# lemerleau/RAFFT

Hardware: AMD Instinct MI355X
Metric: sequences/sec (whole node) on benchmark set, beam N=100; kcal/mol MAE vs CPU (higher is better)
Workload: dtype f32 FFT -> exact int counts, f64 scores, i32 dcal energies

## Files before the change

### rafft_amd/csrc/rafft_device.h

```cpp
#pragma once
#include <hip/hip_runtime.h>
#include <stdint.h>

#define RAFFT_MAX_LEN 32768

struct SmallT {
    int16_t stack[7][7];
    int16_t mmH[7][5][5], mmI[7][5][5], mm1n[7][5][5], mm23[7][5][5], mmM[7][5][5], mmE[7][5][5];
    int16_t d5[7][5], d3[7][5];
    int32_t hairpin[31], bulge[31], interior[31];
    int32_t ml_base, ml_closing, ml_intern, ninio, max_ninio, term_au;
    int32_t lsb, pad_lsb_[3];
    uint32_t sp_key[128]; int32_t sp_e[128];
    uint32_t sp_filter[32];
    int16_t stk4[256];
};
static_assert(sizeof(SmallT) % 16 == 0, "SmallT is copied to LDS in 16-byte pieces");
__host__ __device__ inline uint32_t sp_tag(int size) { return (uint32_t)(size == 3 ? 1 : size == 4 ? 2 : 3) << 28; }
__host__ __device__ inline uint32_t sp_slot(uint32_t tagged) { return (tagged * 2654435761u) >> 25; }
__host__ __device__ inline uint32_t sp_filter_index(int size, int c5, int l5, int l3, int c3)
{
    return ((sp_tag(size) >> 28) << 8) | (uint32_t)((c5 + 3) & 3) | (uint32_t)((l5 + 3) & 3) << 2 | (uint32_t)((l3 + 3) & 3) << 4 | (uint32_t)((c3 + 3) & 3) << 6;
}
struct BigT {
// ... 229 lines not shown

__device__ inline int loop_energy_br(const SmallT *T, const BigT *B, const uint8_t *S, int L, int ci, int cj, const BrList &bl, int &g)
{
    const int k = bl.count();
    if (ci < 0) {
        int e = 0;
        for (int i = 0; i < k; i++) {
            int p, q;
            bl.get(i, p, q);
            e += e_stem(T, pair_type(S[p], S[q]), p > 0 ? (int)S[p - 1] : -1, q < L - 1 ? (int)S[q + 1] : -1, true);
        }
        return e;
    }
    const int type = pair_type(S[ci], S[cj]);
    if (k == 0) return e_hairpin(T, B, cj - ci - 1, type, S, ci, cj);
    if (k == 1) {
        int p, q;
        bl.get(0, p, q);
        return e_intloop(T, B, p - ci - 1, cj - q - 1, type, rtype(pair_type(S[p], S[q])), S[ci + 1], S[cj - 1], S[p - 1], S[q + 1], g);
    }
    int e = 0, u = cj - ci - 1;
    for (int i = 0; i < k; i++) {
        int p, q;
        bl.get(i, p, q);
        e += e_stem(T, pair_type(S[p], S[q]), S[p - 1], S[q + 1], false);
        u -= q - p + 1;
    }
    e += e_stem(T, rtype(type), S[cj - 1], S[ci + 1], false);
    return e + T->ml_closing + u * T->ml_base;
}

struct BrPrefix { const int *pe_ext, *pe_ml; const uint16_t *psp; };
__device__ inline int loop_energy_pre(const SmallT *T, const BigT *B, const uint8_t *S, int L, int ci, int cj, const BrList &bl, const BrPrefix &pf, int &g)
{
    const int k = bl.count();
    if (ci < 0) {
        int e = pf.pe_ext[bl.a1] - pf.pe_ext[bl.a0] + pf.pe_ext[bl.b1] - pf.pe_ext[bl.b0];
        if (bl.has_mid)
            e += e_stem(T, pair_type(S[bl.mp], S[bl.mq]), bl.mp > 0 ? (int)S[bl.mp - 1] : -1, bl.mq < L - 1 ? (int)S[bl.mq + 1] : -1, true);
        return e;
    }
    const int type = pair_type(S[ci], S[cj]);
    if (k == 0) return e_hairpin(T, B, cj - ci - 1, type, S, ci, cj);
    if (k == 1) {
        int p, q;
        bl.get(0, p, q);
        return e_intloop(T, B, p - ci - 1, cj - q - 1, type, rtype(pair_type(S[p], S[q])), S[ci + 1], S[cj - 1], S[p - 1], S[q + 1], g);
    }
    int e = pf.pe_ml[bl.a1] - pf.pe_ml[bl.a0] + pf.pe_ml[bl.b1] - pf.pe_ml[bl.b0];
    int u = cj - ci - 1 - ((int)pf.psp[bl.a1] - (int)pf.psp[bl.a0] + (int)pf.psp[bl.b1] - (int)pf.psp[bl.b0]);
    if (bl.has_mid) {
        e += e_stem(T, pair_type(S[bl.mp], S[bl.mq]), S[bl.mp - 1], S[bl.mq + 1], false);
        u -= bl.mq - bl.mp + 1;
    }
    e += e_stem(T, rtype(type), S[cj - 1], S[ci + 1], false);
    return e + T->ml_closing + u * T->ml_base;
}

__device__ __forceinline__ int br_lower(const uint32_t *br, int nbr, int x)
{
    int lo = 0, hi = nbr;
    while (lo < hi) {
        int mid = (lo + hi) >> 1;
        if ((int)(br[mid] & 0xffffu) < x) lo = mid + 1; else hi = mid;
    }
    return lo;
}

__device__ __forceinline__ void br_lower4(const uint32_t *br, int nbr, int x0, int x1, int x2, int x3, int &r0, int &r1, int &r2, int &r3)
{
    int a = 0, b = 0, c = 0, e = 0;
    int step = nbr > 0 ? 1 << (31 - __clz(nbr)) : 0;
    for (; step > 0; step >>= 1) {
        const int ia = a + step, ib = b + step, ic = c + step, ie = e + step;
        const int va = ia <= nbr ? (int)(br[ia - 1] & 0xffffu) : 0x7fffffff, vb = ib <= nbr ? (int)(br[ib - 1] & 0xffffu) : 0x7fffffff;
        const int vc = ic <= nbr ? (int)(br[ic - 1] & 0xffffu) : 0x7fffffff, ve = ie <= nbr ? (int)(br[ie - 1] & 0xffffu) : 0x7fffffff;
        if (va < x0) a = ia;
        if (vb < x1) b = ib;
        if (vc < x2) c = ic;
        if (ve < x3) e = ie;
    }
    r0 = a; r1 = b; r2 = c; r3 = e;
}
```

### rafft_amd/csrc/rafft_expand.hip

```cpp
#pragma once


__device__ __forceinline__ unsigned long long mask_window(const unsigned long long *X, int W, int start)
{
    if (start >= 64 * W || start <= -64) return 0ULL;
    const int q = start >> 6, bsh = start & 63;
    const unsigned long long lo = (q >= 0 && q < W) ? X[q] : 0ULL;
    const unsigned long long hi = (q + 1 >= 0 && q + 1 < W) ? X[q + 1] : 0ULL;
    return bsh ? (lo >> bsh) | (hi << (64 - bsh)) : lo;
}

template <int NT, class CodeAt>
__device__ inline void build_masks(unsigned long long *F, unsigned long long *R, int W, int n, const CodeAt &code_at, const uint16_t *pos, int tid)
{
    for (int wq = tid >> 6; wq < W; wq += NT / 64) {
        const int t = wq * 64 + (tid & 63);
        const int c0 = t < n ? code_at(t) : 0;
        const unsigned long long bA = __ballot(c0 == 1), bC = __ballot(c0 == 2), bG = __ballot(c0 == 3), bU = __ballot(c0 == 4);
        const unsigned long long bg = __ballot(t >= 1 && t < n && (int)pos[t] - (int)pos[t > 0 ? t - 1 : 0] == 1);
        if ((tid & 63) == 0) { F[0 * W + wq] = bA; F[1 * W + wq] = bC; F[2 * W + wq] = bG; F[3 * W + wq] = bU; F[4 * W + wq] = bg; }
    }
    if (NT == 64) { __builtin_amdgcn_fence(__ATOMIC_ACQ_REL, "wavefront"); __builtin_amdgcn_wave_barrier(); } else __syncthreads();
    for (int idx = tid; idx < 5 * W; idx += NT) {
        const int which = idx / W, w = idx - which * W;
// ... 874 lines not shown
        if (item >= n_items) { fetch_left = 0; continue; }
        const int nid = NT == 64 ? __builtin_amdgcn_readfirstlane(d.work[cls][item]) : d.work[cls][item];
        const int L = d.nd[nid].L;
        const int n = d.nd[nid].n, ci = d.nd[nid].ci, cj = d.nd[nid].cj, nbr = d.nd[nid].nbr;
        const int par_dcal = d.nd[nid].pdcal;
        const uint16_t *posg = d.pos + d.nd[nid].pos;
        const uint32_t *brg = d.br + d.nd[nid].br;
        const uint8_t *codes = d.codes + d.nd[nid].soff;
        const int sx0 = ci < 0 ? 0 : ci, sx1 = ci < 0 ? L : cj + 1;
        const int spad = LONGSEQ ? 0 : (int)((uintptr_t)(codes + sx0) & 3u);
        const uint8_t *Sl = LONGSEQ ? codes : (const uint8_t *)Sl_lds + spad - sx0;
        const int m = 2 * n - 1;
        const int P = next_pow2_ge(m);
        const int logP = 31 - __clz(P);
        const int Pk = LONGSEQ == 2 ? 0 : P;
        const int Kp = d.K < m ? (d.K > 0 ? d.K : 0) : m;
        ExpandRegion<CODE_LDS> g{tm};
        g.nid = nid; g.n = n; g.m = m; g.P = P; g.logP = logP; g.Kp = Kp; g.nbr = nbr; g.ci = ci; g.cj = cj; g.L = L; g.par_dcal = par_dcal;
        g.codes = codes; g.Sl = Sl;

        load_region<NT, LONGSEQ>(d, g, posg, brg, Sl_lds, sx0, sx1, spad);

        const bool direct = (NT == 64) && n <= 64 && !force_fft;
        const bool mw = !direct && LONGSEQ != 2 && (nofft || (n <= d.direct_n && P >= 128 && dbg.lag == nullptr && !force_fft &&
                        d.gc >= 0.0 && d.au >= 0.0 && d.gu >= 0.0));
        const bool ranked = m > Kp;
        const bool selected = ranked && P >= 128;
        const bool inplace = (ranked && !selected) || (dbg.lag != nullptr && !selected);
        const RegionA<LONGSEQ> A(lds, lay, P, Pk, n, nmax, selected, inplace, nofft, d, gteam);
        LagTally tally;
        if (LONGSEQ == 2 || mw) lag_values_masks<NT, PROD>(d, g, A, tally);
        else if (direct) lag_values_wave<NT, PROD>(d, g, A, tally);
        else {
            fft_correlate<NT>(g, A, tw, twN);
            lag_values_fft<NT, PROD>(d, g, A, tally);
        }

        if (selected) {
            select_lags<NT, PROD>(g, A, tally);
            report_ranking<NT>(g, A);
        } else sort_lags_inplace<NT>(g, A);

        const int C = (NT >= 256 && selected) ? max(1, min(8, NT / max(Kp, 1))) : 1;
        const bool ws_masks = PROD || (d.gc >= 0.0 && d.au >= 0.0 && d.gu >= 0.0 && !force_fft);
        if (ws_masks) {
            const int W = A.W();
            unsigned long long *F = A.slide_masks(), *R = F + MASK_F_WORDS * W;
            WsPart *parts = A.slide_parts();
            if (LONGSEQ != 2 && (!mw || A.inplace)) {
                build_masks<NT>(F, R, W, n, [&](int t) -> int { return g.code_at(t); }, pos, tid);
                ESYNC();
            }
            const uint32_t *F32 = (const uint32_t *)F, *R32 = (const uint32_t *)R;
            const int W2 = 2 * W;
            double wgc = d.gc, wau = d.au, wgu = d.gu;
            asm volatile("" : "+v"(wgc), "+v"(wau), "+v"(wgu));
            auto win = [](const uint32_t *X, int start) -> uint32_t { const int q_ = start >> 5; return __builtin_amdgcn_alignbit(X[q_ + 1], X[q_], (uint32_t)(start & 31)); };
            for (int q = tid; q < Kp * C; q += NT) {
                const int r = q / C, c = q - r * C;
                const int lagp = rk[r];
                const Diag dg = diag_of(lagp, n);
                const int ip0 = dg.ip0;
                const int lim = eligible_prefix(pos, dg.len, dg.len2, ip0, dg.jp0, d.min_hp);
                const int ca = (int)((long long)lim * c / C), ce = (int)((long long)lim * (c + 1) / C);
                const int rs0 = n - 1 - lagp + ip0;
                auto cells = [&](int k, uint32_t &pGC, uint32_t &pAU, uint32_t &pGU, uint32_t &cm) {
                    const int cs = ip0 + 32 * k, rs = rs0 + 32 * k;
                    const uint32_t fA = win(F32 + 0 * W2, cs), fC = win(F32 + 1 * W2, cs), fG = win(F32 + 2 * W2, cs), fU = win(F32 + 3 * W2, cs);
                    const uint32_t xA = win(R32 + 0 * W2, rs), xC = win(R32 + 1 * W2, rs), xG = win(R32 + 2 * W2, rs), xU = win(R32 + 3 * W2, rs);
                    pGC = d.gc != 0.0 ? ((fG & xC) | (fC & xG)) : 0u;
                    pAU = d.au != 0.0 ? ((fA & xU) | (fU & xA)) : 0u;
                    pGU = d.gu != 0.0 ? ((fG & xU) | (fU & xG)) : 0u;
                    cm = win(F32 + 4 * W2, cs) & win(R32 + 4 * W2, rs);
                    if (k == 0) cm &= ~1u;
                };
                auto span = [](int lo_, int hi_, int cb) -> uint32_t {
                    uint32_t m_ = ~0u;
                    if (lo_ > cb) m_ &= ~0u << (lo_ - cb);
                    if (hi_ < cb + 32) m_ &= (1u << (hi_ - cb)) - 1u;
                    return m_;
                };
                double mx_s = 0.0, prev = 0.0;
                int mx_nb = 0, mx_c = 0, last_c = -2, runlen = 0, mx_i = 0, mx_j = 0;
                if (ce > ca) {
                    int z = ca;
                    if (ca > 0) {
                        for (int kz = (ca - 1) >> 5;; kz--) {
                            const int cb = kz << 5;
                            uint32_t pGC, pAU, pGU, cm;
                            cells(kz, pGC, pAU, pGU, cm);
                            const uint32_t zeros = ~(pGC | pAU | pGU) & span(0, ca, cb);
                            if (zeros) { z = cb + 32 - __clz((int)zeros); break; }
                            if (cb == 0) { z = 0; break; }
                        }
                    }
                    for (int k = z >> 5; k <= (ce - 1) >> 5; k++) {
                        const int cb = k << 5;
                        uint32_t pGC, pAU, pGU, cm;
                        cells(k, pGC, pAU, pGU, cm);
                        uint32_t any = (pGC | pAU | pGU) & span(z, ce, cb);
                        while (any) {
                            const int bi = __ffs((int)any) - 1;
                            any &= any - 1u;
                            const int cc = cb + bi;
                            const double w8 = ((pGC >> bi) & 1u) ? wgc : ((pAU >> bi) & 1u) ? wau : wgu;
                            if (cc != last_c + 1) { prev = 0.0; runlen = 0; }
                            double t = w8;
                            if ((cm >> bi) & 1u) t = (prev + w8) * w8;
                            runlen++;
                            if ((C == 1 || cc >= ca) && t >= mx_s) { mx_s = t; mx_nb = runlen; mx_c = cc; }
                            prev = t; last_c = cc;
                        }
                    }
                    if (mx_nb == 0) mx_c = ce - 1;
                    mx_i = ip0 + mx_c; mx_j = lagp - mx_i;
                }
                if (C == 1) store_slide(g, r, mx_nb, mx_i, mx_j, mx_s);
                else { WsPart wp; wp.score = mx_s; wp.nb = mx_nb; wp.mi = mx_i; wp.mj = mx_j; wp.any = ce > ca ? 1 : 0; parts[q] = wp; }
            }
            if (C > 1) merge_slide_parts<NT>(g, parts, C);
        } else window_slide_cells<NT>(d, g, A, C);
        ESYNC();

        const BrPrefix pf = branch_prefix_sums<NT>(g, A);
        stems_dE<NT>(d, g, pf);
        if constexpr (NT == 64) emit_wave(d, g, A, shard, slab_base, slab_left, st);
        else emit_team<NT>(d, g, A, shard, slab_base, slab_left, st);
    }
    if (tid == 0 && st.items) {
        Counters::StatLine *sl = &d.c->xstat[cls][gteam & (NSHARD - 1)];
        flush_stats(sl, st.items, st.n, st.lags, st.nbr);
    }
    if (tid == 0 && misc[24]) {
        Counters::StatLine *sl = &d.c->xstat[cls][gteam & (NSHARD - 1)];
        flush_guess_stats(sl, misc[24], misc[25], misc[26]);
    }
}
```

### rafft_amd/csrc/rafft_expand_small.hip

```cpp
#pragma once

template <int TL> struct SmLds {
    static constexpr int NL = 2 * TL;
    static constexpr int off_S = 0;
    static constexpr int off_pos = SM_SPAN + 8;
    static constexpr int off_br = off_pos + 2 * TL;
    static constexpr int off_pe = off_br + 4 * TL;
    static constexpr int off_psp = off_pe + 8 * (TL + 1);
    static constexpr int off_ck = (off_psp + 2 * (TL + 1) + 7) & ~7;
    static constexpr int off_val = off_ck + 8 * NL;
    static constexpr int per_team = (off_val + 8 * NL + 15) & ~15;
};
#define SM_GUARD 4608
static_assert(sizeof(SmallT) <= SM_GUARD, "energy tables must fit the guard area");
#define SM_WG_WAVES 4
template <int TL> constexpr int small_lds_bytes() { return SM_GUARD + SM_WG_WAVES * (64 / TL) * SmLds<TL>::per_team; }

#ifndef RAFFT_SMALL_WAVES
#define RAFFT_SMALL_WAVES 4
#endif

__device__ __forceinline__ uint32_t sm_shift(uint32_t x, int s)
{
    return s >= 0 ? (s < 32 ? x >> s : 0u) : (s > -32 ? x << -s : 0u);
// ... 34 lines not shown
    if (gw == 0 && lane == 0) d.c->n_mat = 0;
    const int shard = gw & (NSHARD - 1);
    unsigned long long st_items = 0, st_n = 0, st_lags = 0, st_nbr = 0;
    unsigned int st_eval = 0, st_guess = 0, st_kguess = 0;
    const unsigned FETCH = n_items > 4u * TPW * n_waves ? (unsigned)d.fetch_bulk : 1u;
    unsigned fetch_base = 0, fetch_left = 0;
    const FetchPlan fplan = fetch_plan(d, n_items, FETCH * TPW, TPW);
    int fshard = (int)(gw & (NSHARD - 1));
    unsigned long long ffailed = 0;
    unsigned long long slab_base = 0; unsigned slab_left = 0;
    const bool dbg = !PROD && d.dbg.lag != nullptr;
    const double par_none = 0.0; (void)par_none;

    for (;;) {
        wave_sync();
        if (fetch_left == 0) {
            unsigned fcount = TPW;
            fetch_base = fetch_chunk(d, cls, fplan, fshard, ffailed, fcount);
            if (fetch_base == ~0u) break;
            fetch_left = fcount / TPW;
        }
        const unsigned item0 = fetch_base;
        fetch_base += TPW; fetch_left--;
        if (item0 >= n_items) { fetch_left = 0; continue; }
        const bool act = item0 + (unsigned)tq < n_items;
        const int nid = d.work[cls][act ? item0 + tq : item0];
        const NodeRec *nr = &d.nd[nid];
        const int n = nr->n, ci = nr->ci, cj = nr->cj, nbr = nr->nbr, L = nr->L, par_dcal = nr->pdcal;
        const uint16_t *posg = d.pos + nr->pos;
        const uint32_t *brg = d.br + nr->br;
        const uint8_t *codes = d.codes + nr->soff;
        const int sx0 = ci < 0 ? 0 : ci;
        const uint8_t *Sl = (const uint8_t *)Sw - sx0;
        const int m = 2 * n - 1;

        int myp = -1, c = 0;
        if (act && tl < n) {
            const int p = posg[tl];
            myp = p & 0x0FFF; c = p >> 12;
            pos[tl] = (uint16_t)myp;
            Sw[myp - sx0] = (uint8_t)c;
        }
        if (act && tl < nbr) {
            const uint32_t u = brg[tl];
            brl[tl] = u & 0x0FFF0FFFu;
            Sw[(int)(u & 0x0FFFu) - sx0] = (uint8_t)((u >> 12) & 0xFu);
            Sw[(int)((u >> 16) & 0x0FFFu) - sx0] = (uint8_t)(u >> 28);
        }
        if (act && ci >= 0 && tl < 2) { const int x = tl ? cj : ci; Sw[x - sx0] = codes[x]; }
        const uint32_t px_ = row16_or((uint32_t)((c + 3) & 3) << (2 * (tl & 15)));
        const unsigned long long p2 = (unsigned long long)(uint32_t)__shfl((int)px_, tbase + 15, 64) |
                                      (TL == 32 ? (unsigned long long)(uint32_t)__shfl((int)px_, tbase + 31, 64) << 32 : 0ULL);
        const unsigned long long bA = __ballot(c == 1), bC = __ballot(c == 2), bG = __ballot(c == 3), bU = __ballot(c == 4);
        const int pprev = __shfl_up(myp, 1, TL);
        const unsigned long long bg = __ballot(act && tl >= 1 && tl < n && myp - pprev == 1);
        const uint32_t mA = (uint32_t)(bA >> tbase) & TM, mC = (uint32_t)(bC >> tbase) & TM, mG = (uint32_t)(bG >> tbase) & TM,
                       mU = (uint32_t)(bU >> tbase) & TM, mg = (uint32_t)(bg >> tbase) & TM;
        const int rs = 32 - n;
        const uint32_t rA = __brev(mA) >> rs, rC = __brev(mC) >> rs, rG = __brev(mG) >> rs, rU = __brev(mU) >> rs, rg = __brev(mg) >> rs;
        wave_sync();
        double wgc = d.gc, wau = d.au, wgu = d.gu;
        asm volatile("" : "+v"(wgc), "+v"(wau), "+v"(wgu));

        int w_nb[2], w_mi[2], w_mj[2];
        double w_sc[2];
#pragma unroll
        for (int s = 0; s < 2; s++) {
            const int k = tl + s * TL;
            int mx_nb = 0, mx_i = 0, mx_j = 0;
            double mx_s = 0.0;
            if (act && k < m) {
                const int len = k < n ? k + 1 : 2 * n - k - 1;
                const int len2 = (len >> 1) + (len & 1);
                const int ip0 = k < n ? 0 : k - n + 1, jp0 = k < n ? k : n - 1;
                const int lim = eligible_prefix(pos, len, len2, ip0, jp0, d.min_hp);
                if (lim > 0) {
                    const int sft = n - 1 - k;
                    const uint32_t xA = sm_shift(rA, sft), xC = sm_shift(rC, sft), xG = sm_shift(rG, sft), xU = sm_shift(rU, sft);
                    const uint32_t pGC = d.gc != 0.0 ? ((mG & xC) | (mC & xG)) : 0u;
                    const uint32_t pAU = d.au != 0.0 ? ((mA & xU) | (mU & xA)) : 0u;
                    const uint32_t pGU = d.gu != 0.0 ? ((mG & xU) | (mU & xG)) : 0u;
                    const uint32_t cm = mg & sm_shift(rg, sft - 1) & ~(1u << ip0);
                    const uint32_t range = (lim >= 32 ? ~0u : ((1u << lim) - 1u)) << ip0;
                    uint32_t any = (pGC | pAU | pGU) & range;
                    double prev = 0.0;
                    int last_ip = -2, runlen = 0;
                    bool found = false;
                    while (any) {
                        const int ip = __ffs((int)any) - 1;
                        any &= any - 1;
                        const uint32_t bit = 1u << ip;
                        const double w8 = (pGC & bit) ? wgc : (pAU & bit) ? wau : wgu;
                        if (ip != last_ip + 1) { prev = 0.0; runlen = 0; }
                        double t = w8;
                        if (cm & bit) t = (prev + w8) * w8;
                        runlen++;
                        if (t >= mx_s) { mx_s = t; mx_nb = runlen; mx_i = ip; mx_j = k - ip; found = true; }
                        prev = t; last_ip = ip;
                    }
                    if (!found) { mx_i = ip0 + lim - 1; mx_j = k - mx_i; }
                }
            }
            w_nb[s] = mx_nb; w_mi[s] = mx_i; w_mj[s] = mx_j; w_sc[s] = mx_s;
        }

        int w_k[2] = {tl, tl + TL};
        if (!dbg) {
            const unsigned long long sb0 = __ballot(w_nb[0] > 0) & tmask, sb1 = __ballot(w_nb[1] > 0) & tmask;
            const int n0 = __popcll(sb0), nst = n0 + __popcll(sb1);
            uint32_t *sl = (uint32_t *)ck;
            if (w_nb[0] > 0) sl[__popcll(sb0 & lt_lane)] = (uint32_t)w_nb[0] | ((uint32_t)w_mi[0] << 8) | ((uint32_t)tl << 16);
            if (w_nb[1] > 0) sl[n0 + __popcll(sb1 & lt_lane)] = (uint32_t)w_nb[1] | ((uint32_t)w_mi[1] << 8) | ((uint32_t)(tl + TL) << 16);
            wave_sync();
#pragma unroll
            for (int s = 0; s < 2; s++) {
                const int idx = tl + s * TL;
                const uint32_t e = idx < nst ? sl[idx] : 0u;
                w_nb[s] = (int)(e & 255u); w_mi[s] = (int)((e >> 8) & 255u); w_k[s] = (int)(e >> 16); w_mj[s] = w_k[s] - w_mi[s];
            }
            wave_sync();
        }
        {
            int ve = 0, vm = 0, vs = 0;
            if (act && tl < nbr) {
                const uint32_t u = brl[tl];
                const int p = (int)(u & 0xffffu), q = (int)(u >> 16);
                const int tt = pair_type(Sl[p], Sl[q]);
                if (ci < 0) ve = e_stem(T, tt, p > 0 ? (int)Sl[p - 1] : -1, q < L - 1 ? (int)Sl[q + 1] : -1, true);
                vm = e_stem(T, tt, p > 0 ? (int)Sl[p - 1] : 0, q < L - 1 ? (int)Sl[q + 1] : 0, false);
                vs = q - p + 1;
            }
            int xe = ve, xm = vm, xs = vs;
#pragma unroll
            for (int o = 1; o < TL; o <<= 1) {
                const int ye = __shfl_up(xe, o, TL), ym = __shfl_up(xm, o, TL), ys = __shfl_up(xs, o, TL);
                if (tl >= o) { xe += ye; xm += ym; xs += ys; }
            }
            if (act && tl < nbr) { pe_ext[tl] = xe - ve; pe_ml[tl] = xm - vm; psp[tl] = (uint16_t)(xs - vs); }
            if (act && tl == (nbr > 0 ? nbr - 1 : 0)) {
                if (nbr > 0) { pe_ext[nbr] = xe; pe_ml[nbr] = xm; psp[nbr] = (uint16_t)xs; }
                else { pe_ext[0] = 0; pe_ml[0] = 0; psp[0] = 0; }
            }
        }
        wave_sync();
        const double par_e = dcal_to_energy(par_dcal);
        const BrPrefix pf{pe_ext, pe_ml, psp};
        int w_dd[2];
        bool w_keep[2];
        {
            const bool anystem = act && (w_nb[0] > 0 || w_nb[1] > 0);
            int e_old = 0, g_old = 0;
            if (anystem) {
                const BrList all_br{brl, 0, nbr, 0, 0, 0, 0, 0};
                e_old = loop_energy_pre(T, B, Sl, L, ci, cj, all_br, pf, g_old);
            }
#pragma unroll
            for (int s = 0; s < 2; s++) {
                w_dd[s] = 0; w_keep[s] = false;
                const int nb = w_nb[s];
                if (act && nb > 0) {
                    int g = g_old;
                    const int mi = w_mi[s], mj = w_mj[s];
                    const int a0 = pos[mi], b0 = pos[mj], ao = pos[mi - nb + 1], bo = pos[mj + nb - 1];
                    int lo, hi, lo_o, hi_o;
                    br_lower4(brl, nbr, a0, b0, ao, bo, lo, hi, lo_o, hi_o);
                    BrList outer{brl, 0, lo_o, hi_o, nbr, 1, ao, bo};
                    int e_new = loop_energy_pre(T, B, Sl, L, ci, cj, outer, pf, g);
                    BrList inner{brl, lo, hi, 0, 0, 0, 0, 0};
                    e_new += loop_energy_pre(T, B, Sl, L, a0, b0, inner, pf, g);
                    if (nb <= 16 && a0 - ao == nb - 1 && bo - b0 == nb - 1)
                        e_new += stem_stack_windows(T, (uint32_t)(p2 >> (2 * (mi - nb + 1))), (uint32_t)(p2 >> (2 * mj)), nb);
                    else {
                    int pa = a0, pb = b0, ty_in = pair_type(Sl[a0], Sl[b0]);
                    for (int t = 1; t < nb; t++) {
                        const int a = pos[mi - t], b = pos[mj + t];
                        const int ty = pair_type(Sl[a], Sl[b]);
                        if (pa == a + 1 && pb == b - 1)
                            e_new += T->stack[ty][rtype(ty_in)];
                        else {
                            const int lo2 = br_lower(brl, nbr, a), hi2 = br_lower(brl, nbr, b);
                            BrList mid{brl, lo2, lo, hi, hi2, 1, pa, pb};
                            e_new += loop_energy_pre(T, B, Sl, L, a, b, mid, pf, g);
// ... 110 lines not shown
```

### rafft_amd/csrc/rafft_kernels.h

```cpp
#pragma once
#include "rafft_device.h"

struct alignas(16) Cand {
    int32_t ddcal;
    uint16_t mi, mj, nb, cut_hi;
    uint32_t cut_lo;
    uint64_t h1, h2;
    __host__ __device__ void set_cuts(int lo0, int hi0, int loo, int hio)
    {
        const unsigned long long v = (unsigned long long)lo0 | ((unsigned long long)hi0 << 12) | ((unsigned long long)loo << 24) | ((unsigned long long)hio << 36);
        cut_lo = (uint32_t)v; cut_hi = (uint16_t)(v >> 32);
    }
    __host__ __device__ void get_cuts(int &lo0, int &hi0, int &loo, int &hio) const
    {
        const unsigned long long v = (unsigned long long)cut_lo | ((unsigned long long)cut_hi << 32);
        lo0 = (int)(v & 4095); hi0 = (int)((v >> 12) & 4095); loo = (int)((v >> 24) & 4095); hio = (int)((v >> 36) & 4095);
    }
};
static_assert(sizeof(Cand) == 32, "Cand must be 32 bytes");

#define NSHARD 64
#ifndef SEEN0
#define SEEN0 8192
#endif
static_assert(SEEN0 >= 2048 && (SEEN0 & (SEEN0 - 1)) == 0, "seen tables are powers of two >= 2048 slots (their bitmaps start on whole words)");
#define NCLS 6
#define NGEN 4
struct ShardCtr { unsigned long long v; unsigned long long pad[7]; };

struct alignas(128) StRec {
    int32_t seq, dcal, node0, nnodes, parent, nprod;
    int32_t c0d, nsp;
    uint64_t h1, h2;
    uint64_t sp, cursor, combo, total, prod;
    uint64_t c0h1, c0h2;
    uint64_t pad2[3];
};
static_assert(sizeof(StRec) == 128, "StRec is two cache lines");

struct alignas(64) NodeRec {
    int32_t seq, pdcal, n, ci, cj, nbr, ncand, L;
    uint64_t pos, br, cand, soff;
};
static_assert(sizeof(NodeRec) == 64, "NodeRec must be one cache line");

struct ProdEnt { uint32_t cnt; int32_t node; uint64_t off; };
struct alignas(16) MatRec { int32_t sid, sq, L, dcal, nprod, pad; uint64_t combo, prod, soff; };

struct Counters {
    unsigned int n_mat;
    unsigned int overflow;
    unsigned int n_done;
    unsigned int max_nprod;
    unsigned int pad0_[12];
    unsigned long long n_struct, pad1_[7];
    unsigned long long trec_n, tsid_top, pad2_[6];
    unsigned long long seen_top, pad3_[7];
    struct WorkCtr { unsigned int v; unsigned int pad[15]; } n_work[NCLS];
    unsigned long long n_expand, sum_n, sum_lags, n_children, sum_struct_len, n_alias, sum_nbr;
    unsigned long long cls_items[NCLS], cls_sum_n[NCLS], cls_sum_lags[NCLS];
    ShardCtr node[NSHARD], pos[NSHARD], br[NSHARD], sp[NSHARD], cand[NSHARD], node_prev[NSHARD], prod[NSHARD];
    ShardCtr nlist[NSHARD];
    ShardCtr wcur[NCLS][NSHARD];
    unsigned long long wdone[NCLS];
    unsigned long long wdone_pad[8 - NCLS];
    struct StatLine { unsigned long long items, n, lags, nbr, alias, children, struct_len, evals, guessed, kept_guessed, pad[6]; } xstat[NCLS][NSHARD];
};

enum { OVF_STRUCT = 1, OVF_NODE = 2, OVF_POS = 4, OVF_SP = 8, OVF_CAND = 16, OVF_SEEN = 32,
       OVF_TRAJ = 64, OVF_WORK = 128, OVF_PROD = 256, OVF_SORT = 512, OVF_BR = 1024, OVF_LOOPTAB = 2048, OVF_PRODLIST = 4096 };

struct DebugOut {
    int *n_ranked, *lag, *nb, *mi, *mj, *ddcal, *kept;
    double *corval, *score;
};

struct Dev {
    const EnergyTables *T;
    const float2 *tw;
    int S;
    const uint8_t *codes;
    const int *seq_off, *seq_len;
    int K, B, max_branch, min_hp, traj, memo, force_fft, rl_cap, mat_tile, merge_cls;
    double *big_keyv; size_t big_stride;
    int max_prod;
    int fetch_bulk, taper_pct;
    int direct_n;
    int sm_n4, sm_n5;
    int cand_slab;
    int cls1_P, cls1_br;
    int c3_switch;
    double min_nrj, gc, au, gu;
    int *beam, *beam_n, *done, *nsteps;
    int ch_cap;
    uint16_t *ch_parent; uint64_t *ch_combo; int *ch_dcal; uint64_t *ch_h;
    uint64_t *seen; uint64_t seen_cap_total;
    uint64_t *seen_off; uint32_t *seen_cap, *seen_cnt;
    uint32_t *seen_bm;
    uint32_t *seen_mode;
    uint32_t seen_bm0;
    uint32_t st_cap;
    StRec *st;
    ProdEnt *prod; uint64_t prod_shard_cap;
    uint32_t nd_cap;
    uint64_t nd_base, nd_shard_cap, pos_base, pos_shard_cap, br_shard_cap, sp_shard_cap, cand_shard_cap;
    NodeRec *nd;
    int *nlist;
    unsigned long long *cslot;
    uint32_t *nd_slot;
    unsigned long long *looptab; uint64_t looptab_cap;
    uint16_t *pos; uint64_t pos_cap;
    int pos_packed;
    uint32_t *br; uint64_t br_cap;
    uint32_t *sp; uint64_t sp_cap;
    Cand *cand; uint64_t cand_cap;
    int4 *trec; uint32_t trec_cap;
    int *tsid; uint64_t tsid_cap;
    int *work[NCLS]; uint32_t work_cap;
    MatRec *mat; uint32_t mat_cap;
    Counters *c;
    DebugOut dbg;
};

#define CLS0_P 4096
#define CLS1_P 512
#define CLS01_L 1280
#define CLS1_BR 256
#define CLS2_P 2048
#define MAX_P 8192
#define MAX_BR 1024
#define BIG_BR 4095
#define BIG_N 32768
#define LDS_SEQ 4096
#define MAX_PROD 64
#define MAX_PROD_LONG 1024
#define RL_CAP 1024

__host__ __device__ inline int next_pow2_ge(int x) { int p = 2; while (p < x) p <<= 1; return p; }
#define SM_SPAN 448
__host__ __device__ inline int node_class(int n, int span, int nbr, int merge_cls = 0, int cls1_P = CLS1_P, int cls1_br = CLS1_BR,
                                          int K = 0, int sm_n4 = 0, int sm_n5 = 0)
{
    if (merge_cls == 0 && n >= 2 && n <= sm_n5 && 2 * n - 1 <= K && span <= SM_SPAN) {
        if (n <= sm_n4 && nbr <= 16) return 4;
        if (sm_n5 > sm_n4 && nbr <= 32) return 5;
    }
    int P = next_pow2_ge(2 * n - 1);
    if (P > MAX_P || nbr > MAX_BR) return 0;
    if (merge_cls == 3) return 3;
    if (merge_cls == 2) return P <= CLS2_P ? 2 : 3;
    if (span <= CLS01_L && P <= cls1_P && nbr <= cls1_br) return 1;
    if (P <= CLS2_P) return 2;
    return 3;
}

#define MASK_F_WORDS 5
#define MASK_WORDS 10
struct ExpandLds {
    int offA, szA, off_pos, off_code, off_p2, off_S, off_br, off_rk, off_nb, off_mi, off_mj, off_dd, off_keep, off_w, off_misc,
        per_team,
        off_tab, off_tw,
        total;
};
__host__ __device__ inline ExpandLds expand_lds(int Pmax, int Lmax, int nmax, int brmax, int Kmax, bool tab_lds, int wpb = 1, bool nofft = false, int nt = 512,
                                                bool code_lds = true)
{
    ExpandLds l;
    auto al = [](int x) { return (x + 15) & ~15; };
    l.offA = 0;
    l.szA = al(16 * Pmax);
    if (nofft) {
        const int need1 = 8 * Pmax + 8 * MASK_WORDS * ((nmax + 63) / 64) + 8 + (nt > 64 && 24 * nt > 1152 ? 24 * nt : 1152) , need2 = 8 * Pmax + 10 * (brmax + 1) + 16, need3 = 8 * Pmax + 8 * Kmax + 64;
        l.szA = al(need1 > need2 ? (need1 > need3 ? need1 : need3) : (need2 > need3 ? need2 : need3));
    }
    int o = l.szA;
// ... 25 lines not shown
```

### rafft_amd/csrc/rafft_wave.h

```cpp
#pragma once

namespace {

hipEvent_t next_event(std::vector<hipEvent_t> &used)
{
    hipEvent_t e = nullptr;
    if (!g.ev_free.empty()) { e = g.ev_free.back(); g.ev_free.pop_back(); }
    else if (hipEventCreate(&e) != hipSuccess) return nullptr;
    used.push_back(e);
    return e;
}

struct Span { hipEvent_t a, b; int kind; };
static int g_span_level = 1;
static inline bool span_on(int kind) { return g_span_level >= 2 || (g_span_level == 1 && kind == 11); }
#define SPAN_REC(ev, st, kind) do { if (span_on(kind)) HIPCHK(hipEventRecord((ev), (st))); } while (0)

struct HostOut {
    std::vector<rafft_seq_result> seq;
    std::vector<std::vector<int>> step_size, step_off;
    std::vector<int> one_size, one_off;
    std::vector<const char *> db_ptr;
    std::vector<const int *> dcal_ptr;
    std::vector<std::shared_ptr<struct PinChunk>> chunks;
// ... 106 lines not shown

int Wave::setup()
{
    S = seqs.size();
    tw0 = std::chrono::steady_clock::now();
    if (cfg.test_hard_fail >= 0 && (int)S == cfg.test_hard_fail) return fail(RAFFT_ERR_PARAM, "test hook: hard failure of this wave");
    off.resize(S); len.resize(S);
    sumL = 0;
    for (size_t i = 0; i < S; i++) { off[i] = (int)sumL; len[i] = seqs[i].len; sumL += seqs[i].len; }
    const size_t st_codes = 0, st_off = (sumL + 16 + 63) & ~(size_t)63, st_len = st_off + ((S * 4 + 63) & ~(size_t)63),
                 st_ctr = st_len + ((S * 4 + 63) & ~(size_t)63), st_soff = st_ctr + ((sizeof(Counters) + 63) & ~(size_t)63),
                 st_scap = st_soff + ((S * 8 + 63) & ~(size_t)63), st_bytes = st_scap + S * 4;
    stage = pin_acquire(st_bytes);
    if (!stage.p) return fail(RAFFT_ERR_HIP, "hipHostMalloc failed for the input staging buffer");
    uint8_t *codes = (uint8_t *)stage.p + st_codes;
    for (size_t i = 0; i < S; i++) {
        uint8_t *dst = codes + off[i];
        if (seqs[i].c) memcpy(dst, seqs[i].c, (size_t)seqs[i].len);
        else {
            const unsigned char *src = (const unsigned char *)seqs[i].s;
            for (int x = 0; x < seqs[i].len; x++) dst[x] = kBaseCode[src[x]] & 7;
        }
    }
    memset(codes + sumL, 0, 16);
    memcpy((char *)stage.p + st_off, off.data(), S * 4);
    memcpy((char *)stage.p + st_len, len.data(), S * 4);
    const double ms_enc = since(tw0);
    int maxL = 0;
    for (size_t i = 0; i < S; i++) maxL = std::max(maxL, len[i]);
    const int direct_n_ = cfg.direct_n;
    const bool force_fft_ = cfg.force_fft != 0;
    const bool nofft1 = !seam && !force_fft_ && direct_n_ >= cls1_P(cfg) / 2 && p.gc_wei >= 0.0 && p.au_wei >= 0.0 && p.gu_wei >= 0.0;
    const bool nofft2 = nofft1 && direct_n_ >= CLS2_P / 2;
    if (int rc = class_cfg(cfg, p.nb_mode, maxL, cf, nofft1, nofft2, nofft1)) return rc;
    if (cfg.trace)
        for (int c = 0; c < NGEN; c++)
            fprintf(stderr, "[rafft] expand class %d: %d threads x %d regions per workgroup, P <= %d, branches <= %d, lags <= %d, LDS %d B%s\n", c, cf[c].nt, cf[c].wpb,
                    cf[c].Pmax, cf[c].brmax, cf[c].Kmax, cf[c].lds, cf[c].nofft ? " (no FFT buffers)" : "");
    merge_target = maxL > CLS2_P / 2 ? 3 : 2;
    JobPlan jp = plan_job(cfg, p, seqs, est);
    seen_cap0 = std::move(jp.seen_cap0);
    seen0_total = jp.seen0_total;
    const double seen0_avg = jp.seen0_avg;
    c = jp.caps;
    if (std::max((size_t)c.sort_cap * 8, (size_t)24 * 1024) + RL_CAP * 12 + (size_t)(p.max_stack + 4) * (sizeof(ParentInfo) + 16) + 1024 > 150 * 1024)
        return fail(RAFFT_ERR_PARAM, "max_branch + 2*max_stack too large for the LDS-resident beam sort");
    B = (size_t)p.max_stack;

    size_t Sr = S;
    Caps cr = c;
    if (S < merge_cap() && !seam) {
        const double reserve_frac = cfg.reserve_frac;
        const size_t tries[2] = {S >= 256 ? merge_cap() : std::max<size_t>(S, std::min<size_t>(64, 32 * S)), S >= 256 ? std::min(merge_cap(), 5 * S) : S};
        Sr = S;
        for (size_t want : tries) {
            if (want <= S) continue;
            Caps big = plan_caps(cfg, want, (size_t)((double)sumL * (double)want / (double)S), p, est, seen0_avg);
            if (big.bytes <= (size_t)((double)g.hbm_total * reserve_frac)) { cr = big; Sr = want; break; }
        }
    }
    reserve = (double)Sr / (double)S;
    const size_t sumLr = Sr == S ? sumL : (size_t)((double)sumL * (double)Sr / (double)S);
#define ENS(buf, bytes) do { if (int rc_ = ensure(ws.buf, (bytes))) return rc_; } while (0)
    ENS(codes, sumLr + 16); ENS(seq_off, Sr * 4); ENS(seq_len, Sr * 4);
    ENS(beam, Sr * B * 4); ENS(beam_n, Sr * 4); ENS(done, Sr * 4); ENS(nsteps, Sr * 4);
    ENS(ch_parent, Sr * c.ch_cap * 2); ENS(ch_combo, Sr * c.ch_cap * 8); ENS(ch_dcal, Sr * c.ch_cap * 4); ENS(ch_h, Sr * c.ch_cap * 16);
    ENS(seen, cr.seen * 16); ENS(seen_off, Sr * 8); ENS(seen_cap, Sr * 4); ENS(seen_cnt, Sr * 4); ENS(seen_bm, cr.seen / 8 + 64); ENS(seen_mode, Sr * 4);
    ENS(st, cr.st * sizeof(StRec)); ENS(prod, cr.nd * 16);
    ENS(nd, cr.nd * sizeof(NodeRec)); ENS(nlist, cr.nd * 4); ENS(nd_slot, cr.nd * 4); ENS(cslot, cr.cand * 8);
    ENS(pos, cr.pos * 2); ENS(br, cr.br * 4); ENS(sp, cr.sp * 4); ENS(cand, cr.cand * 32);
    ENS(looptab, cr.looptab * 8);
    ENS(trec, cr.trec * 16); ENS(tsid, cr.tsid * 4);
    ENS(work0, cr.work * 4); ENS(work1, cr.work * 4); ENS(work2, cr.work * 4); ENS(work3, cr.work * 4); ENS(work4, cr.work * 4); ENS(work5, cr.work * 4);
    ENS(mat, cr.mat * sizeof(MatRec));
    ENS(counters, sizeof(Counters));
#undef ENS


    memset(&d, 0, sizeof d);
    d.T = g.T; d.tw = g.tw; d.S = (int)S;
    d.codes = (const uint8_t *)ws.codes.p; d.seq_off = (const int *)ws.seq_off.p; d.seq_len = (const int *)ws.seq_len.p;
    d.K = p.nb_mode; d.B = p.max_stack; d.max_branch = p.max_branch; d.min_hp = p.min_hp; d.traj = p.traj;
    d.min_nrj = p.min_nrj; d.gc = p.gc_wei; d.au = p.au_wei; d.gu = p.gu_wei;
    d.memo = (p.min_nrj == 0.0) ? 1 : 0;
    if (cfg.no_memo) d.memo = 0;
    if (cfg.force_fft) d.force_fft = 1;
    d.rl_cap = RL_CAP;
    longseq = maxL > LDS_SEQ;
    d.pos_packed = longseq ? 0 : 1;
    d.max_prod = (longseq || big_prod) ? MAX_PROD_LONG : MAX_PROD;
    if (cfg.test_max_prod > 0 && !big_prod && !longseq) d.max_prod = std::max(1, std::min(cfg.test_max_prod, MAX_PROD));
    if (longseq) {
        d.big_stride = (size_t)2 * cf[0].nmax + (size_t)2 * cf[0].nmax / 4;
        if (int rc = ensure(ws.big, (size_t)cf[0].grid * d.big_stride * 8)) return rc;
        d.big_keyv = (double *)ws.big.p;
    } else if (cf[3].direct3) {
        d.big_stride = (size_t)MAX_P + (size_t)MAX_P / 4;
        if (int rc = ensure(ws.big, (size_t)cf[3].grid * d.big_stride * 8)) return rc;
        d.big_keyv = (double *)ws.big.p;
    }
    d.cls1_P = cls1_P(cfg); d.cls1_br = cf[1].brmax;
    d.c3_switch = cfg.c3_switch >= 0 ? cfg.c3_switch : g.n_cu;
    d.cand_slab = std::max(16, cfg.slab);
    d.fetch_bulk = std::max(1, cfg.fetch);
    d.taper_pct = std::max(0, std::min(100, cfg.taper));
    d.direct_n = cfg.direct_n;
    d.sm_n4 = std::max(0, std::min(cfg.small_n4, 16)); d.sm_n5 = std::max(d.sm_n4, std::min(cfg.small_n5, 32));
    if (!d.pos_packed || d.force_fft || !(p.gc_wei >= 0.0 && p.au_wei >= 0.0 && p.gu_wei >= 0.0)) d.sm_n4 = d.sm_n5 = 0;
    d.mat_tile = 64;
    d.mat_tile = std::max(1, std::min(cfg.mat_tile, 64));
    if (cfg.rl_cap >= 0) d.rl_cap = std::min(cfg.rl_cap, RL_CAP);
    d.beam = (int *)ws.beam.p; d.beam_n = (int *)ws.beam_n.p; d.done = (int *)ws.done.p; d.nsteps = (int *)ws.nsteps.p;
    d.ch_cap = c.ch_cap;
    d.ch_parent = (uint16_t *)ws.ch_parent.p; d.ch_combo = (uint64_t *)ws.ch_combo.p; d.ch_dcal = (int *)ws.ch_dcal.p; d.ch_h = (uint64_t *)ws.ch_h.p;
    d.seen = (uint64_t *)ws.seen.p; d.seen_cap_total = c.seen;
    d.seen_off = (uint64_t *)ws.seen_off.p; d.seen_cap = (uint32_t *)ws.seen_cap.p; d.seen_cnt = (uint32_t *)ws.seen_cnt.p;
    d.seen_bm = (uint32_t *)ws.seen_bm.p; d.seen_mode = (uint32_t *)ws.seen_mode.p;
    d.st_cap = (uint32_t)c.st;
    d.st = (StRec *)ws.st.p;
    d.prod = (ProdEnt *)ws.prod.p; d.prod_shard_cap = c.nd / NSHARD;
    d.nd_cap = (uint32_t)c.nd;
    d.nd = (NodeRec *)ws.nd.p; d.nlist = (int *)ws.nlist.p; d.nd_slot = (uint32_t *)ws.nd_slot.p; d.cslot = (unsigned long long *)ws.cslot.p;
    d.looptab = (unsigned long long *)ws.looptab.p; d.looptab_cap = c.looptab;
    d.pos = (uint16_t *)ws.pos.p; d.pos_cap = c.pos; d.br = (uint32_t *)ws.br.p; d.br_cap = c.br;
    d.sp = (uint32_t *)ws.sp.p; d.sp_cap = c.sp;
    d.cand = (Cand *)ws.cand.p; d.cand_cap = c.cand;
    d.trec = (int4 *)ws.trec.p; d.trec_cap = (uint32_t)c.trec; d.tsid = (int *)ws.tsid.p; d.tsid_cap = c.tsid;
    d.work[0] = (int *)ws.work0.p; d.work[1] = (int *)ws.work1.p; d.work[2] = (int *)ws.work2.p; d.work[3] = (int *)ws.work3.p;
    d.work[4] = (int *)ws.work4.p; d.work[5] = (int *)ws.work5.p; d.work_cap = (uint32_t)c.work;
    d.mat = (MatRec *)ws.mat.p; d.mat_cap = (uint32_t)c.mat;
    d.c = (Counters *)ws.counters.p;
    d.nd_base = S; d.nd_shard_cap = (c.nd - S) / NSHARD;
    d.pos_base = sumL; d.pos_shard_cap = (c.pos - sumL) / NSHARD;
    d.sp_shard_cap = c.sp / NSHARD;
    d.br_shard_cap = c.br / NSHARD; d.cand_shard_cap = c.cand / NSHARD;
    if (seam) d.dbg = seam->dbg;


    for (int v = 1; v >= 0; v--) {
        const size_t nt = v ? 1024 : 256;
        const size_t rest = RL_CAP * 12 + B * sizeof(ParentInfo) + (B + 1) * 8 + ((B + 3) & ~(size_t)3) * 4 + 128 + B * 4;
        size_t bm = v ? 32768 : 4096;
        if (cfg.seen_bm_max >= 0) bm = std::min((size_t)cfg.seen_bm_max & ~(size_t)15, 32 * nt);
        while (bm && 24 * nt + bm + rest > 160 * 1024) bm = (bm / 2) & ~(size_t)15;
        if (v == 0) bm = std::min(bm, bs_bm[1]);
        bs_bm[v] = bm;
        bs_lds[v] = std::max((size_t)c.sort_cap * 8, 24 * nt + bm) + rest;
    }
    d.seen_bm0 = (uint32_t)bs_bm[S < (size_t)std::max(0, cfg.wide_below) ? 1 : 0];

    const double ms_plan = since(tw0);
    hipStream_t st = ws.stream;
    double t_mark = ms_plan;
    auto slow_call = [&](const char *what) {
        if (!cfg.trace) return;
        const double now = since(tw0);
        if (now - t_mark > 1.0) fprintf(stderr, "[rafft] setup of a wave of %zu sequences: %s kept the host for %.3f ms\n", S, what, now - t_mark);
        t_mark = now;
    };
    memset(&hc, 0, sizeof hc);
    hc.n_struct = S; hc.seen_top = seen0_total;
    memcpy((char *)stage.p + st_ctr, &hc, sizeof hc);
    {
        uint64_t *so = (uint64_t *)((char *)stage.p + st_soff);
        uint32_t *sc = (uint32_t *)((char *)stage.p + st_scap);
        size_t o = 0;
// ... 354 lines not shown
```

Measured before the change: 572,600.

## Resolve isolated stacking cells with bitmask ranking in window-score scans

After: 567,300. Within noise of the previous version (-0.9%).

```diff
diff --git a/rafft_amd/csrc/rafft_device.h b/rafft_amd/csrc/rafft_device.h
--- a/rafft_amd/csrc/rafft_device.h
+++ b/rafft_amd/csrc/rafft_device.h
@@ -335,3 +335,46 @@
     }
     r0 = a; r1 = b; r2 = c; r3 = e;
 }
+
+__host__ __device__ inline uint32_t ws_iso_ranks(double gc, double au, double gu)
+{
+    const double w[3] = {gc, au, gu};
+    double v[6];
+    for (int t = 0; t < 3; t++) { v[2 * t] = w[t]; v[2 * t + 1] = (0.0 + w[t]) * w[t]; }
+    uint32_t ranks = 0;
+    for (int c = 0; c < 6; c++) {
+        uint32_t r = 0;
+        for (int e = 0; e < 6; e++) r += v[e] > v[c] ? 1u : 0u;
+        ranks |= r << (3 * c);
+    }
+    return ranks;
+}
+struct WsIso { uint32_t iso, loop, cont; int cell; double score; };
+__host__ __device__ __forceinline__ WsIso ws_isolated(uint32_t pGC, uint32_t pAU, uint32_t pGU, uint32_t cm, uint32_t span, bool prev_pairs,
+                                                      bool has_next, uint32_t ranks, double wgc, double wau, double wgu)
+{
+    WsIso r;
+    const uint32_t p = (pGC | pAU | pGU) & span;
+    r.cont = cm & p & ((p << 1) | (prev_pairs ? 1u : 0u));
+    r.loop = p & (r.cont | (r.cont >> 1) | (has_next ? 0x80000000u : 0u));
+    r.iso = p & ~r.loop;
+    const uint32_t pt[3] = {pGC, pAU, pGU};
+    uint32_t key = ~0u;
+#pragma unroll
+    for (int c = 0; c < 6; c++) {
+        const uint32_t m = r.iso & pt[c >> 1] & ((c & 1) ? cm : ~cm);
+        const uint32_t kc = (uint32_t)(m ? __builtin_clz(m) : -1) | (((ranks >> (3 * c)) & 7u) << 5);
+        key = kc < key ? kc : key;
+    }
+    r.cell = key == ~0u ? -1 : 31 - (int)(key & 31u);
+    const uint32_t bit = key == ~0u ? 0u : 0x80000000u >> (key & 31u);
+    const double w8 = (pGC & bit) ? wgc : (pAU & bit) ? wau : wgu;
+    r.score = !bit ? 0.0 : (cm & bit) ? (0.0 + w8) * w8 : w8;
+    return r;
+}
+__host__ __device__ __forceinline__ int ws_run_ending_at(uint32_t p, int bi)
+{
+    const uint32_t x = ~p << (31 - bi);
+    const int nz = x ? __builtin_clz(x) : 32;
+    return nz < bi + 1 ? nz : bi + 1;
+}
diff --git a/rafft_amd/csrc/rafft_expand.hip b/rafft_amd/csrc/rafft_expand.hip
--- a/rafft_amd/csrc/rafft_expand.hip
+++ b/rafft_amd/csrc/rafft_expand.hip
@@ -980,6 +980,45 @@
                 };
                 double mx_s = 0.0, prev = 0.0;
                 int mx_nb = 0, mx_c = 0, last_c = -2, runlen = 0, mx_i = 0, mx_j = 0;
+                if constexpr (NT == 64) {
+                    (void)last_c; (void)runlen;
+                    if (ce > 0) {
+                        const int kl = (ce - 1) >> 5;
+                        uint32_t p_last = 0u;
+                        mx_c = -1;
+                        for (int k = 0; k <= kl; k++) {
+                            const int cb = k << 5;
+                            uint32_t pGC, pAU, pGU, cm;
+                            cells(k, pGC, pAU, pGU, cm);
+                            const uint32_t sp = span(0, ce, cb);
+                            const WsIso wi = ws_isolated(pGC, pAU, pGU, cm, sp, (p_last >> 31) != 0u, k < kl, d.ws_rank, wgc, wau, wgu);
+                            uint32_t any = wi.loop;
+                            while (any) {
+                                const int bi = __ffs((int)any) - 1;
+                                any &= any - 1u;
+                                const double w8 = ((pGC >> bi) & 1u) ? wgc : ((pAU >> bi) & 1u) ? wau : wgu;
+                                double t = w8;
+                                if ((cm >> bi) & 1u) t = ((((wi.cont >> bi) & 1u) ? prev : 0.0) + w8) * w8;
+                                if (t >= mx_s) { mx_s = t; mx_c = cb + bi; }
+                                prev = t;
+                            }
+                            if (wi.cell >= 0 && (wi.score > mx_s || (wi.score == mx_s && cb + wi.cell > mx_c))) { mx_s = wi.score; mx_c = cb + wi.cell; }
+                            p_last = (pGC | pAU | pGU) & sp;
+                        }
+                        if (mx_c >= 0) {
+                            int kw = mx_c >> 5, bi = mx_c & 31;
+                            uint32_t pw = p_last;
+                            for (bool have = kw == kl;; have = false) {
+                                if (!have) { uint32_t pGC, pAU, pGU, cm; cells(kw, pGC, pAU, pGU, cm); pw = pGC | pAU | pGU; }
+                                const int run = ws_run_ending_at(pw, bi);
+                                mx_nb += run;
+                                if (run <= bi || kw == 0) break;
+                                kw--; bi = 31;
+                            }
+                        } else mx_c = ce - 1;
+                        mx_i = ip0 + mx_c; mx_j = lagp - mx_i;
+                    }
+                } else
                 if (ce > ca) {
                     int z = ca;
                     if (ca > 0) {
diff --git a/rafft_amd/csrc/rafft_expand_small.hip b/rafft_amd/csrc/rafft_expand_small.hip
--- a/rafft_amd/csrc/rafft_expand_small.hip
+++ b/rafft_amd/csrc/rafft_expand_small.hip
@@ -140,22 +140,23 @@
                     const uint32_t pGU = d.gu != 0.0 ? ((mG & xU) | (mU & xG)) : 0u;
                     const uint32_t cm = mg & sm_shift(rg, sft - 1) & ~(1u << ip0);
                     const uint32_t range = (lim >= 32 ? ~0u : ((1u << lim) - 1u)) << ip0;
-                    uint32_t any = (pGC | pAU | pGU) & range;
+                    const WsIso wi = ws_isolated(pGC, pAU, pGU, cm, range, false, false, d.ws_rank, wgc, wau, wgu);
+                    uint32_t any = wi.loop;
                     double prev = 0.0;
-                    int last_ip = -2, runlen = 0;
-                    bool found = false;
+                    int mx_ip = -1;
                     while (any) {
                         const int ip = __ffs((int)any) - 1;
                         any &= any - 1;
                         const uint32_t bit = 1u << ip;
                         const double w8 = (pGC & bit) ? wgc : (pAU & bit) ? wau : wgu;
-                        if (ip != last_ip + 1) { prev = 0.0; runlen = 0; }
                         double t = w8;
-                        if (cm & bit) t = (prev + w8) * w8;
-                        runlen++;
-                        if (t >= mx_s) { mx_s = t; mx_nb = runlen; mx_i = ip; mx_j = k - ip; found = true; }
-                        prev = t; last_ip = ip;
+                        if (cm & bit) t = (((wi.cont & bit) ? prev : 0.0) + w8) * w8;
+                        if (t >= mx_s) { mx_s = t; mx_ip = ip; }
+                        prev = t;
                     }
+                    if (wi.cell >= 0 && (wi.score > mx_s || (wi.score == mx_s && wi.cell > mx_ip))) { mx_s = wi.score; mx_ip = wi.cell; }
+                    const bool found = mx_ip >= 0;
+                    if (found) { mx_nb = ws_run_ending_at((pGC | pAU | pGU) & range, mx_ip); mx_i = mx_ip; mx_j = k - mx_ip; }
                     if (!found) { mx_i = ip0 + lim - 1; mx_j = k - mx_i; }
                 }
             }
diff --git a/rafft_amd/csrc/rafft_kernels.h b/rafft_amd/csrc/rafft_kernels.h
--- a/rafft_amd/csrc/rafft_kernels.h
+++ b/rafft_amd/csrc/rafft_kernels.h
@@ -91,6 +91,7 @@
     int cls1_P, cls1_br;
     int c3_switch;
     double min_nrj, gc, au, gu;
+    uint32_t ws_rank;
     int *beam, *beam_n, *done, *nsteps;
     int ch_cap;
     uint16_t *ch_parent; uint64_t *ch_combo; int *ch_dcal; uint64_t *ch_h;
diff --git a/rafft_amd/csrc/rafft_wave.h b/rafft_amd/csrc/rafft_wave.h
--- a/rafft_amd/csrc/rafft_wave.h
+++ b/rafft_amd/csrc/rafft_wave.h
@@ -212,6 +212,7 @@
     d.codes = (const uint8_t *)ws.codes.p; d.seq_off = (const int *)ws.seq_off.p; d.seq_len = (const int *)ws.seq_len.p;
     d.K = p.nb_mode; d.B = p.max_stack; d.max_branch = p.max_branch; d.min_hp = p.min_hp; d.traj = p.traj;
     d.min_nrj = p.min_nrj; d.gc = p.gc_wei; d.au = p.au_wei; d.gu = p.gu_wei;
+    d.ws_rank = ws_iso_ranks(d.gc, d.au, d.gu);
     d.memo = (p.min_nrj == 0.0) ? 1 : 0;
     if (cfg.no_memo) d.memo = 0;
     if (cfg.force_fft) d.force_fft = 1;
```
